# delldu/TransMVSNet

Hardware: AMD Instinct MI355X
Metric: depth maps/sec @ DTU 864x1152 N=5 (48/32/8 hyp); Abs depth L1 vs ref (higher is better)
Workload: dtype f32; 1 GPU; DTU 864x1152, N=5 views, cascade 48/32/8, B=1, hot path from FeatureNet outputs (FMT+pathway+stage glue+cost volume+CostRegNet+softmax/WTA); global_batch=1, parallelism=replica1, launch=hip_graph replay

## Files before the change

### transmvsnet_amd/csrc/common.h

```cpp
#pragma once

#include <hip/hip_runtime.h>
#include <stdint.h>

#include "../../include/transmvs.h"

#define TMVS_CHECK_LAUNCH()                                   \
  do {                                                        \
    hipError_t _e = hipGetLastError();                        \
    if (_e != hipSuccess) return TMVS_ERR_HIP;                \
  } while (0)

namespace tmvs {

constexpr int kWave = 64;

__device__ __forceinline__ float relu(float x) { return x > 0.f ? x : 0.f; }

__device__ __forceinline__ bool xcd_range_tap(int ntaps, int nblk, int& rb, int& k) {
  const int per = 8 * ntaps;
  const int grp = blockIdx.x / per, within = blockIdx.x % per;
  k = within / 8;
  rb = grp * 8 + within % 8;
  return rb < nblk;
}
static inline dim3 xcd_range_tap_grid(int ntaps, int nblk) { return dim3((unsigned)((nblk + 7) / 8 * 8 * ntaps)); }

__device__ __forceinline__ void chunk_row_coords(long v, int H, int W, int& b, int& y, int& x) {
  const long vl = v & ~63L;
  const unsigned lo = __builtin_amdgcn_readfirstlane((unsigned)vl);
  const unsigned hi = __builtin_amdgcn_readfirstlane((unsigned)((unsigned long)vl >> 32));
  const long vb = (long)(((unsigned long)hi << 32) | lo);
  const long t = vb / W;
  x = (int)(vb - t * W) + (int)(v - vb);
  y = (int)(t % H);
  b = (int)(t / H);
  while (x >= W) {
    x -= W;
    if (++y == H) {
      y = 0;
      ++b;
    }
  }
}

__device__ __forceinline__ void chunk_row_coords3(long v, int D, int H, int W, int& b, int& z, int& y, int& x) {
  const long vl = v & ~63L;
  const unsigned lo = __builtin_amdgcn_readfirstlane((unsigned)vl);
  const unsigned hi = __builtin_amdgcn_readfirstlane((unsigned)((unsigned long)vl >> 32));
  const long vb = (long)(((unsigned long)hi << 32) | lo);
  long t = vb / W;
  x = (int)(vb - t * W) + (int)(v - vb);
  y = (int)(t % H);
  t /= H;
  z = (int)(t % D);
  b = (int)(t / D);
  while (x >= W) {
    x -= W;
    if (++y == H) {
      y = 0;
      if (++z == D) {
        z = 0;
        ++b;
      }
    }
  }
}

template <int OFF>
__device__ __forceinline__ int xor_lane_dpp(int v) {
  if constexpr (OFF == 1) return __builtin_amdgcn_mov_dpp(v, 0xB1, 0xF, 0xF, false);
  else if constexpr (OFF == 2) return __builtin_amdgcn_mov_dpp(v, 0x4E, 0xF, 0xF, false);
  else if constexpr (OFF == 4)
    return __builtin_amdgcn_mov_dpp(__builtin_amdgcn_mov_dpp(v, 0x141, 0xF, 0xF, false), 0x1B, 0xF, 0xF, false);
  else if constexpr (OFF == 8)
    return __builtin_amdgcn_mov_dpp(__builtin_amdgcn_mov_dpp(v, 0x140, 0xF, 0xF, false), 0x141, 0xF, 0xF, false);
  else if constexpr (OFF == 16) return __builtin_amdgcn_ds_swizzle(v, 0x1F | (16 << 10));
  else return __shfl_xor(v, 32, 64);
}
template <int OFF>
__device__ __forceinline__ double xor_add_dpp(double x) {
  const int lo = xor_lane_dpp<OFF>(__double2loint(x)), hi = xor_lane_dpp<OFF>(__double2hiint(x));
  return x + __hiloint2double(hi, lo);
}
__device__ __forceinline__ double wave_xor_sum_dpp(double x) {
  x = xor_add_dpp<32>(x);
  x = xor_add_dpp<16>(x);
  x = xor_add_dpp<8>(x);
  x = xor_add_dpp<4>(x);
  x = xor_add_dpp<2>(x);
  return xor_add_dpp<1>(x);
}

template <typename T>
__device__ __forceinline__ double strided_sum(const T* __restrict__ p, long j0, long n, long step, size_t stride,
                                              double s) {
  constexpr int kBatch = 8;
  long j = j0;
  for (; j + (kBatch - 1) * step < n; j += kBatch * step) {
    T t[kBatch];
#pragma unroll
    for (int u = 0; u < kBatch; ++u) t[u] = p[(size_t)(j + u * step) * stride];
#pragma unroll
    for (int u = 0; u < kBatch; ++u) s += (double)t[u];
  }
  for (; j < n; j += step) s += (double)p[(size_t)j * stride];
  return s;
}

__device__ __forceinline__ int xcd_remap(int bid, int nblk) {
  const int xcd = bid & 7;
  const int q = nblk >> 3, r = nblk & 7;
  const int base = (xcd < r) ? xcd * (q + 1) : r * (q + 1) + (xcd - r) * q;
  return base + (bid >> 3);
}

constexpr int kRsrcWord3 = 0x00020000;
constexpr unsigned kOffOut = 0x80000000u;
__device__ __forceinline__ __amdgpu_buffer_rsrc_t raw_rsrc(const void* base, unsigned bytes) {
  return __builtin_amdgcn_make_buffer_rsrc(const_cast<void*>(base), (short)0, (int)bytes, kRsrcWord3);
}
__device__ __forceinline__ float buf_load_f32(__amdgpu_buffer_rsrc_t r, unsigned off) {
  return __uint_as_float(__builtin_amdgcn_raw_buffer_load_b32(r, (int)off, 0, 0));
}
typedef float floatx4_t __attribute__((ext_vector_type(4)));
__device__ __forceinline__ floatx4_t buf_load_f32x4(__amdgpu_buffer_rsrc_t r, unsigned off) {
  return __builtin_bit_cast(floatx4_t, __builtin_amdgcn_raw_buffer_load_b128(r, (int)off, 0, 0));
}

template <int D, typename PutProb>
__device__ __forceinline__ int softmax_first_max(const float (&x)[D], PutProb put_prob, float& best) {
  float m = x[0];
#pragma unroll
  for (int d = 1; d < D; ++d) m = fmaxf(m, x[d]);
  float s = 0.f;
#pragma unroll
  for (int d = 0; d < D; ++d) s = s + expf(x[d] - m);
  const float lse = logf(s);
  best = -1.f;
  int bi = 0;
#pragma unroll
  for (int d = 0; d < D; ++d) {
    const float pr = expf((x[d] - m) - lse);
    put_prob(d, pr);
    if (pr > best) {
      best = pr;
      bi = d;
    }
  }
  return bi;
}

}
```

### transmvsnet_amd/csrc/costreg.hip

```cpp
#include "common.h"

#include <utility>

namespace tmvs {

typedef float floatx4 __attribute__((ext_vector_type(4)));

struct Vec4 {
  float v[4];
  __device__ __forceinline__ void load(const float* p) {
    const float4 t = *reinterpret_cast<const float4*>(p);
    v[0] = t.x;
    v[1] = t.y;
    v[2] = t.z;
    v[3] = t.w;
  }
  __device__ __forceinline__ void zero() { v[0] = v[1] = v[2] = v[3] = 0.f; }
};

struct Buf {
  __amdgpu_buffer_rsrc_t r;
  __device__ __forceinline__ Buf(const float* base, uint32_t nbytes)
      : r(__builtin_amdgcn_make_buffer_rsrc(const_cast<float*>(base), (short)0, (int)nbytes, 0x00020000)) {}
  static constexpr int kOOB = (int)0x80000000u;
// ... 261 lines not shown
  auto chunk = [&](int ch, auto more_c) {
    constexpr bool MORE = decltype(more_c)::value;
    if (MORE && KDSKIP && kd_lo > kd_hi) fetch(ch + 1);
    if constexpr (KDSKIP) {
#pragma unroll 1
      for (int kd = kd_lo; kd <= kd_hi; ++kd)
#pragma unroll
        for (int k9 = 0; k9 < 9; ++k9) {
          if (k9 + 2 < 9) {
            wload(ch, kd * 9 + k9 + 2, aw[(k9 + 2) % 3]);
          } else {
            if (kd < kd_hi)
              wload(ch, kd * 9 + k9 + 2, aw[(k9 + 2) % 3]);
            else if (MORE)
              wload(ch + 1, kd_lo * 9 + k9 - 7, aw[(k9 + 2) % 3]);
          }
          if (MORE && k9 == 6 && kd == kd_hi) fetch(ch + 1);
          if (k9 == 0) bload(kd, k9 / 3, k9 % 3, bw[k9 & 1]);
          if (k9 + 1 < 9) bload(kd, (k9 + 1) / 3, (k9 + 1) % 3, bw[(k9 + 1) & 1]);
          tap_mfma(aw[k9 % 3], bw[k9 & 1]);
        }
    } else {
#pragma unroll
      for (int tap = 0; tap < 27; ++tap) {
        if (tap + 2 < 27)
          wload(ch, tap + 2, aw[(tap + 2) % 3]);
        else if (MORE)
          wload(ch + 1, tap - 25, aw[(tap + 2) % 3]);
        if (MORE && tap == 24) fetch(ch + 1);
        if (tap == 0) bload(tap / 9, (tap / 3) % 3, tap % 3, bw[tap & 1]);
        if (tap + 1 < 27) bload((tap + 1) / 9, ((tap + 1) / 3) % 3, (tap + 1) % 3, bw[(tap + 1) & 1]);
        tap_mfma(aw[tap % 3], bw[tap & 1]);
      }
    }
    if (MORE) {
      __syncthreads();
      commit();
      __syncthreads();
    }
  };
#pragma unroll 1
  for (int ch = 0; ch + 1 < NCH; ++ch) chunk(ch, std::true_type{});
  chunk(NCH - 1, std::false_type{});
  }
  const int ow = ow0 + col;
  if (ow >= g.Wo) return;
  const size_t out_n = (size_t)n * g.Do * g.Ho * g.Wo;
#pragma unroll
  for (int m = 0; m < MBW; ++m) {
    const int co = (mb0 + m) * 16 + kgrp * 4;
    const float4 al = *reinterpret_cast<const float4*>(alpha + co);
    const float4 sh = *reinterpret_cast<const float4*>(shift + co);
#pragma unroll
    for (int r = 0; r < NBW; ++r) {
      const int rr = rg * NBW + r;
      const int od = od0 + rr / TH, oh = oh0 + rr % TH;
      if (od >= g.Do || oh >= g.Ho) continue;
      *reinterpret_cast<float4*>(y + (out_n + ((size_t)od * g.Ho + oh) * g.Wo + ow) * COUT + co) =
          bn_act4(acc[r][m], al, sh, g.lo);
    }
  }
}

template <int CIN, int COUT, int TDI, int THI>
__global__ __launch_bounds__(256) void deconv3d_lds_kernel(const float* __restrict__ x,
                                                           const float* __restrict__ wpk,
                                                           const float* __restrict__ alpha,
                                                           const float* __restrict__ shift,
                                                           const float* __restrict__ skip, float* __restrict__ y,
                                                           Geo g) {
  constexpr int CK = 16, PL = 4;
  constexpr int MG = COUT / 16;
  constexpr int NBW = TDI * THI / 4;
  constexpr int LW = 17, LH = THI + 1, LD = TDI + 1;
  constexpr int NVOX = LD * LH * LW;
  static_assert((TDI * THI) % 4 == 0, "tile");
  static_assert(CIN % 16 == 0 && COUT % 16 == 0, "16-channel input chunks, 16-channel output blocks");
  __shared__ __attribute__((aligned(16))) float tile[NVOX * 16];
  __shared__ __attribute__((aligned(16))) float wts[27 * 16 * 16];

  const int nws = (g.Wi + 15) / 16, nhs = (g.Hi + THI - 1) / THI, nds = (g.Di + TDI - 1) / TDI;
  const int wg = xcd_remap(blockIdx.x, gridDim.x);
  const int mg = wg % MG;
  const TileCoord c = tile_coord(wg / MG, nws, nhs, nds, THI, TDI);
  const int n = c.n, mw0 = c.w0, mh0 = c.h0, md0 = c.d0;
  const int lane = threadIdx.x & 63, wv = threadIdx.x >> 6;
  const int col = lane & 15, kgrp = lane >> 4;
  const size_t in_n = (size_t)n * g.Di * g.Hi * g.Wi;

  floatx4 acc[NBW][8];
#pragma unroll
  for (int r = 0; r < NBW; ++r)
#pragma unroll
    for (int cls = 0; cls < 8; ++cls) acc[r][cls] = floatx4{0.f, 0.f, 0.f, 0.f};

#pragma unroll 1
  for (int ch = 0; ch < CIN / CK; ++ch) {
    if (ch) __syncthreads();
    for (int idx = threadIdx.x; idx < NVOX * PL; idx += 256) {
      const int vox = idx / PL, q = idx - vox * PL;
      const int lw = vox % LW, rest = vox / LW, lh = rest % LH, ld = rest / LH;
      const int iw = mw0 + lw, ih = mh0 + lh, id = md0 + ld;
      float4 v = make_float4(0.f, 0.f, 0.f, 0.f);
      if (iw < g.Wi && ih < g.Hi && id < g.Di)
        v = *reinterpret_cast<const float4*>(x + (in_n + ((size_t)id * g.Hi + ih) * g.Wi + iw) * CIN + ch * CK + 4 * q);
      *reinterpret_cast<float4*>(swz16(tile, vox, q)) = v;
    }
    stage_weights16<COUT, CIN>(wts, wpk, mg * 16, ch * CK);
    __syncthreads();
#pragma unroll
    for (int cls = 0; cls < 8; ++cls) {
#pragma unroll
      for (int i = 0; i < deconv_class_taps(cls); ++i) {
        const DeconvTap t = deconv_class_tap(cls, i);
        Vec4 a;
        a.load(swz16(wts + t.tap * 256, col, kgrp));
#pragma unroll
        for (int r = 0; r < NBW; ++r) {
          const int rr = wv * NBW + r;
          const int mdl = rr / THI, mhl = rr - mdl * THI;
          Vec4 b;
          const int lvox = ((mdl + (t.off >> 2)) * LH + mhl + ((t.off >> 1) & 1)) * LW + col + (t.off & 1);
          b.load(swz16(tile, lvox, kgrp));
#pragma unroll
          for (int j = 0; j < PL; ++j)
            acc[r][cls] = __builtin_amdgcn_mfma_f32_16x16x4f32(a.v[j], b.v[j], acc[r][cls], 0, 0, 0);
        }
      }
    }
  }
  const size_t out_n = (size_t)n * g.Do * g.Ho * g.Wo;
  const int mw = mw0 + col;
  if (mw >= g.Wi) return;
  const int co = mg * 16 + kgrp * 4;
  const float4 al = *reinterpret_cast<const float4*>(alpha + co);
  const float4 sh = *reinterpret_cast<const float4*>(shift + co);
#pragma unroll
  for (int r = 0; r < NBW; ++r) {
    const int rr = wv * NBW + r;
    const int md = md0 + rr / THI, mh = mh0 + rr % THI;
    if (md >= g.Di || mh >= g.Hi) continue;
#pragma unroll
    for (int cls = 0; cls < 8; ++cls) {
      const int od = 2 * md + (cls >> 2), oh = 2 * mh + ((cls >> 1) & 1), ow = 2 * mw + (cls & 1);
      const size_t o = (out_n + ((size_t)od * g.Ho + oh) * g.Wo + ow) * COUT + co;
      const float4 s = skip ? *reinterpret_cast<const float4*>(skip + o) : make_float4(0.f, 0.f, 0.f, 0.f);
      *reinterpret_cast<float4*>(y + o) = add4(s, bn_act4(acc[r][cls], al, sh, g.lo));
    }
  }
}

constexpr int kDChunk = 8;

constexpr int kProbCols = 62;
typedef float float2_v __attribute__((ext_vector_type(2)));

__device__ __forceinline__ float lane_from_left(float v) {
  return __int_as_float(__builtin_amdgcn_update_dpp(0, __float_as_int(v), 0x138, 0xF, 0xF, false));
}
__device__ __forceinline__ float lane_from_right(float v) {
  return __int_as_float(__builtin_amdgcn_update_dpp(0, __float_as_int(v), 0x130, 0xF, 0xF, false));
}

__global__ __launch_bounds__(256) void conv0_kernel(const float* __restrict__ x, float* __restrict__ y, int D, int H,
                                                    int W, const float* __restrict__ wt,
                                                    const float* __restrict__ alpha,
                                                    const float* __restrict__ shift, float lo) {
  const int HW = H * W;
  const int nseg = (W + kProbCols - 1) / kProbCols, nrow = (H + 3) / 4, ndc = (D + kDChunk - 1) / kDChunk;
  int lb = xcd_remap(blockIdx.x, gridDim.x);
  const int seg = lb % nseg;
  lb /= nseg;
  const int rowb = lb % nrow;
  lb /= nrow;
  const int dc = lb % ndc;
  const int n = lb / ndc;
  const int lane = threadIdx.x & 63;
  const int h = rowb * 4 + (threadIdx.x >> 6);
  if (h >= H) return;
  const int w = seg * kProbCols + lane - 1;
  const bool writes = lane >= 1 && lane <= kProbCols && w < W;
  const int d0 = dc * kDChunk, d1 = min(D, d0 + kDChunk);
  const __amdgpu_buffer_rsrc_t rx = raw_rsrc(x + (size_t)n * D * HW, (unsigned)(D * HW * 4));
  float* yp = y + ((size_t)n * D * HW + (size_t)h * W + w) * 8;
  const unsigned offw = (unsigned)w < (unsigned)W ? (unsigned)w * 4u : kOffOut;
  unsigned offh[3];
#pragma unroll
  for (int k = 0; k < 3; ++k) offh[k] = (unsigned)(h - 1 + k) < (unsigned)H ? (unsigned)((h - 1 + k) * W) * 4u : kOffOut;
  auto load_raw = [&](int d, float (&o)[3]) {
    const unsigned offd = (unsigned)d < (unsigned)D ? (unsigned)d * (unsigned)HW * 4u : kOffOut;
#pragma unroll
    for (int kh = 0; kh < 3; ++kh) {
      const unsigned off = offd | offh[kh] | offw;
      o[kh] = buf_load_f32(rx, (offd + offh[kh] + offw) | (off & kOffOut));
    }
  };
  auto expand = [&](const float (&r)[3], float (&o)[3][3]) {
#pragma unroll
    for (int kh = 0; kh < 3; ++kh) {
      o[kh][0] = lane_from_left(r[kh]);
      o[kh][1] = r[kh];
      o[kh][2] = lane_from_right(r[kh]);
    }
  };
  float al[8], sh[8];
#pragma unroll
  for (int c = 0; c < 8; ++c) {
    al[c] = alpha[c];
    sh[c] = shift[c];
  }
  float win[3][3][3];
  auto step = [&](int d, float (&raw)[3]) {
    expand(raw, win[2]);
    load_raw(d + 2, raw);
    const float* wk = wt;
    float2_v a[4] = {{0.f, 0.f}, {0.f, 0.f}, {0.f, 0.f}, {0.f, 0.f}};
#pragma unroll
    for (int t = 0; t < 27; ++t) {
      const float xv = win[t / 9][(t / 3) % 3][t % 3];
#pragma unroll
      for (int cp = 0; cp < 4; ++cp)
        a[cp] = __builtin_elementwise_fma(*reinterpret_cast<const float2_v*>(wk + t * 8 + 2 * cp), float2_v{xv, xv},
                                          a[cp]);
    }
    float o[8];
#pragma unroll
    for (int cp = 0; cp < 4; ++cp) {
      o[2 * cp] = act(fmaf(a[cp].x, al[2 * cp], sh[2 * cp]), lo);
      o[2 * cp + 1] = act(fmaf(a[cp].y, al[2 * cp + 1], sh[2 * cp + 1]), lo);
    }
    if (writes) {
      float4* q = reinterpret_cast<float4*>(yp + (size_t)d * HW * 8);
      q[0] = make_float4(o[0], o[1], o[2], o[3]);
      q[1] = make_float4(o[4], o[5], o[6], o[7]);
    }
#pragma unroll
    for (int kh = 0; kh < 3; ++kh)
#pragma unroll
      for (int k = 0; k < 3; ++k) {
        win[0][kh][k] = win[1][kh][k];
        win[1][kh][k] = win[2][kh][k];
      }
  };
  float ra[3];
  load_raw(d0 - 1, ra);
  expand(ra, win[0]);
  load_raw(d0, ra);
  expand(ra, win[1]);
  load_raw(d0 + 1, ra);
  for (int d = d0; d < d1; ++d) step(d, ra);
}


template <int NR, typename Emit>
__device__ __forceinline__ void prob_walk_rows(__amdgpu_buffer_rsrc_t rx, int w, int h, int D, int H, int W, int d0,
                                               const float* __restrict__ wt, Emit emit) {
  constexpr int NL = NR + 2;
  d0 = __builtin_amdgcn_readfirstlane(d0);
  const unsigned offw = (unsigned)w < (unsigned)W ? (unsigned)w * 32u : kOffOut;
  auto load_plane = [&](int i, float4 (&o)[NL][2]) {
#pragma unroll
    for (int j = 0; j < NL; ++j) {
      const int ih = h - 1 + j;
      const unsigned offr = ((unsigned)i < (unsigned)D && (unsigned)ih < (unsigned)H)
                                ? ((unsigned)i * (unsigned)H + (unsigned)ih) * (unsigned)W * 32u
                                : kOffOut;
      const unsigned off = (offr + offw) | ((offr | offw) & kOffOut);
      const floatx4 u = buf_load_f32x4(rx, off);
      const floatx4 v = buf_load_f32x4(rx, off + 16u);
      o[j][0] = make_float4(u[0], u[1], u[2], u[3]);
      o[j][1] = make_float4(v[0], v[1], v[2], v[3]);
    }
  };
  float2_v c12[NR];
#pragma unroll
  for (int r = 0; r < NR; ++r) c12[r] = float2_v{0.f, 0.f};
  auto plane = [&](int i, const float4 (&p)[NL][2]) {
    float acc_next[NR];
#pragma unroll
    for (int r = 0; r < NR; ++r) acc_next[r] = 0.f;
#pragma unroll
    for (int kh = 0; kh < 3; ++kh) {
      int wo = kh * 72;
      asm volatile("" : "+s"(wo));
      const float* wk = wt + __builtin_amdgcn_readfirstlane(wo);
#pragma unroll
      for (int r = 0; r < NR; ++r) {
        const int j = r + kh;
        const float xc[8] = {p[j][0].x, p[j][0].y, p[j][0].z, p[j][0].w, p[j][1].x, p[j][1].y, p[j][1].z, p[j][1].w};
#pragma unroll
        for (int kw = 0; kw < 3; ++kw) {
#pragma unroll
          for (int c = 0; c < 8; ++c) {
            const float xv = kw == 0 ? lane_from_left(xc[c]) : kw == 1 ? xc[c] : lane_from_right(xc[c]);
            const float2_v wp = *reinterpret_cast<const float2_v*>(wk + 2 * (kw * 8 + c));
            acc_next[r] = fmaf(wk[48 + kw * 8 + c], xv, acc_next[r]);
            c12[r] = __builtin_elementwise_fma(wp, float2_v{xv, xv}, c12[r]);
          }
        }
        asm volatile("" : "+v"(acc_next[r]), "+v"(c12[r]));
      }
    }
#pragma unroll
    for (int r = 0; r < NR; ++r) {
      if (i - 1 >= d0) emit(r, i - 1, c12[r].y);
      c12[r] = float2_v{acc_next[r], c12[r].x};
    }
  };
  float4 pa[NL][2], pb[NL][2];
  load_plane(d0 - 1, pa);
#pragma unroll
  for (int j = 0; j < kDChunk + 2; j += 2) {
    const int i = d0 - 1 + j;
    load_plane(i + 1, pb);
    plane(i, pa);
    load_plane(i + 2, pa);
    plane(i + 1, pb);
  }
}

template <int NR>
__global__ __launch_bounds__(256) void prob_kernel(const float* __restrict__ x, float* __restrict__ y, int D, int H,
                                                   int W, const float* __restrict__ wt) {
  const int HW = H * W;
  const int nseg = (W + kProbCols - 1) / kProbCols, nrow = (H + 4 * NR - 1) / (4 * NR), ndc = (D + kDChunk - 1) / kDChunk;
  int lb = xcd_remap(blockIdx.x, gridDim.x);
  const int seg = lb % nseg;
  lb /= nseg;
  const int rowb = lb % nrow;
  lb /= nrow;
  const int dc = lb % ndc;
  const int n = lb / ndc;
  const int lane = threadIdx.x & 63;
  const int h = (rowb * 4 + (threadIdx.x >> 6)) * NR;
  if (h >= H) return;
  const int w = seg * kProbCols + lane - 1;
  const bool writes = lane >= 1 && lane <= kProbCols && w < W;
  const int d0 = dc * kDChunk, d1 = min(D, d0 + kDChunk);
  const __amdgpu_buffer_rsrc_t rx = raw_rsrc(x + (size_t)n * D * HW * 8, (unsigned)(D * HW * 32));
  float* yn = y + (size_t)n * D * HW + (size_t)h * W + w;
  prob_walk_rows<NR>(rx, w, h, D, H, W, d0, wt, [&](int r, int d, float v) {
    if (d < d1 && writes && h + r < H) yn[(size_t)d * HW + (size_t)r * W] = v;
  });
}

template <int D, int NR>
__global__ __launch_bounds__(64 * (D / kDChunk)) void prob_wta_rows_kernel(
    const float* __restrict__ x, const float* __restrict__ wt, const float* __restrict__ hyp, int H, int W, float lo,
    float hi, float* __restrict__ prob, float* __restrict__ depth, float* __restrict__ depth_raw,
    float* __restrict__ conf) {
  constexpr int NW = D / kDChunk;
  __shared__ float lg[NR][D * 64];
  const int HW = H * W;
  const int nseg = (W + kProbCols - 1) / kProbCols, nrow = (H + NR - 1) / NR;
  int lb = xcd_remap(blockIdx.x, gridDim.x);
  const int seg = lb % nseg;
  lb /= nseg;
  const int h0 = (lb % nrow) * NR;
  const int n = lb / nrow;
  const int lane = threadIdx.x & 63, wv = threadIdx.x >> 6;
  const int d0 = wv * kDChunk;
  const int w = seg * kProbCols + lane - 1;
  const bool writes = lane >= 1 && lane <= kProbCols && w < W;
  const __amdgpu_buffer_rsrc_t rx = raw_rsrc(x + (size_t)n * D * HW * 8, (unsigned)(D * HW * 32));
  prob_walk_rows<NR>(rx, w, h0, D, H, W, d0, wt, [&](int r, int d, float v) { lg[r][d * 64 + lane] = v; });
  __syncthreads();
  if (!writes) return;
  for (int r = wv; r < NR; r += NW) {
    const int h = h0 + r;
    if (h >= H) break;
    float xl[D];
#pragma unroll
    for (int d = 0; d < D; ++d) xl[d] = lg[r][d * 64 + lane];
    const size_t base = (size_t)n * D * HW + (size_t)h * W + w;
    float best;
    const int bi = softmax_first_max<D>(xl, [&](int d, float pr) { prob[base + (size_t)d * HW] = pr; }, best);
    const size_t o = (size_t)n * HW + (size_t)h * W + w;
    const float dr = hyp[base + (size_t)bi * HW];
    depth_raw[o] = dr;
    depth[o] = fminf(fmaxf(dr, lo), hi);
    conf[o] = best;
  }
}

template <int TD, int TH>
__global__ __launch_bounds__(256) __attribute__((amdgpu_waves_per_eu(2))) void conv3d_c16_kernel(const float* __restrict__ x, const float* __restrict__ wpk,
                                                         const float* __restrict__ alpha,
                                                         const float* __restrict__ shift, float* __restrict__ y, Geo g,
                                                         int ntiles) {
  constexpr int C = 16, PL = 4, NWV = 4, NBW = TD * TH / NWV, NTH = NWV * 64;
  static_assert(TD * TH % NWV == 0, "rows split evenly over the waves");
  constexpr int LW = 18, LH = TH + 2, LD = TD + 2;
  constexpr int NVOX = LD * LH * LW;
  constexpr int NLD = (NVOX * 4 + NTH - 1) / NTH;
  __shared__ __attribute__((aligned(16))) float tile[NVOX * 16];
  __shared__ __attribute__((aligned(16))) float wts[27 * 16 * 16];
  const int nws = (g.Wo + 15) / 16, nhs = (g.Ho + TH - 1) / TH, nds = (g.Do + TD - 1) / TD;
  const int lane = threadIdx.x & 63, wv = threadIdx.x >> 6;
  const int col = lane & 15, kgrp = lane >> 4;
  const TileRange tr(ntiles);
  if (tr.idle()) return;
  auto coord = [&](int t) { return tile_coord(t, nws, nhs, nds, TH, TD); };
  float4 pf[NLD];
  auto fetch = [&](int t) {
    const TileCoord c = coord(t);
    const size_t in_n = (size_t)c.n * g.Di * g.Hi * g.Wi;
#pragma unroll
    for (int k = 0; k < NLD; ++k) {
      const int idx = threadIdx.x + NTH * k;
      const int vox = idx >> 2, q = idx & 3;
      const int lw = vox % LW, rest = vox / LW, lh = rest % LH, ld = rest / LH;
      const int iw = c.w0 - 1 + lw, ih = c.h0 - 1 + lh, id = c.d0 - 1 + ld;
      pf[k] = make_float4(0.f, 0.f, 0.f, 0.f);
      if (vox < NVOX && (unsigned)iw < (unsigned)g.Wi && (unsigned)ih < (unsigned)g.Hi && (unsigned)id < (unsigned)g.Di)
        pf[k] = *reinterpret_cast<const float4*>(x + (in_n + ((size_t)id * g.Hi + ih) * g.Wi + iw) * C + 4 * q);
    }
  };
  auto commit = [&]() {
#pragma unroll
    for (int k = 0; k < NLD; ++k) {
      const int idx = threadIdx.x + NTH * k;
      const int vox = idx >> 2, q = idx & 3;
      if (vox < NVOX) *reinterpret_cast<float4*>(swz16(tile, vox, q)) = pf[k];
    }
  };
  stage_weights16<C, C>(wts, wpk, 0, 0);
  const float4 al = *reinterpret_cast<const float4*>(alpha + kgrp * 4);
  const float4 sh = *reinterpret_cast<const float4*>(shift + kgrp * 4);
  int t = tr.first();
  if (t < tr.end) {
    fetch(t);
    commit();
  }
  __syncthreads();
  for (; t < tr.end; t += tr.step) {
    const TileCoord c = coord(t);
    const int tn = t + tr.step;
    if (tn < tr.end) fetch(tn);
    floatx4 acc[NBW];
#pragma unroll
    for (int r = 0; r < NBW; ++r) acc[r] = floatx4{0.f, 0.f, 0.f, 0.f};
#pragma unroll
    for (int tap = 0; tap < 27; ++tap) {
      const int kd = tap / 9, kh = (tap / 3) % 3, kw = tap % 3;
      Vec4 a;
      a.load(swz16(wts + tap * 256, col, kgrp));
      Vec4 b[NBW];
#pragma unroll
      for (int r = 0; r < NBW; ++r) {
        const int rr = wv * NBW + r;
        const int odl = rr / TH, ohl = rr - odl * TH;
        const int lvox = ((odl + kd) * LH + ohl + kh) * LW + col + kw;
        b[r].load(swz16(tile, lvox, kgrp));
      }
#pragma unroll
      for (int j = 0; j < PL; ++j)
#pragma unroll
        for (int r = 0; r < NBW; ++r)
          acc[r] = __builtin_amdgcn_mfma_f32_16x16x4f32(a.v[j], b[r].v[j], acc[r], 0, 0, 0);
      if (tap % (NBW > 2 ? 3 : 9) == (NBW > 2 ? 2 : 8)) __builtin_amdgcn_sched_barrier(0);
    }
    const int ow = c.w0 + col;
    const size_t out_n = (size_t)c.n * g.Do * g.Ho * g.Wo;
#pragma unroll
    for (int r = 0; r < NBW; ++r) {
      const int rr = wv * NBW + r;
      const int od = c.d0 + rr / TH, oh = c.h0 + rr % TH;
      if (ow >= g.Wo || od >= g.Do || oh >= g.Ho) continue;
      *reinterpret_cast<float4*>(y + (out_n + ((size_t)od * g.Ho + oh) * g.Wo + ow) * C + kgrp * 4) =
          bn_act4(acc[r], al, sh, g.lo);
// ... 460 lines not shown
      constexpr int s1 = s + 1, ch1 = s1 / 14, i1 = s1 % 14;
      constexpr bool next = s1 < 14 * NCH, next0 = next && deconv_stream_tap(0, i1).cls >= 0;
      if constexpr (next0) a[s1 & 1][0].load(wts[ch1] + deconv_stream_tap(0, i1).tap * 256 + woff);
      if constexpr (next) a[s1 & 1][1].load(wts[ch1] + deconv_stream_tap(1, i1).tap * 256 + woff);
      if constexpr (s < 8) bload(1, s);
      if constexpr (s < 8) sk[s] = sb.ld4(so[s]);
      if constexpr (s >= 8 && s < 8 + NLD) fetch1(fn, s - 8);
#pragma unroll
      for (int j = 0; j < PL; ++j) {
        if constexpr (t0.cls >= 0)
          acc[t0.cls] = __builtin_amdgcn_mfma_f32_16x16x4f32(a[s & 1][0].v[j], b[ch][t0.off].v[j], acc[t0.cls], 0, 0, 0);
        acc[t1.cls] = __builtin_amdgcn_mfma_f32_16x16x4f32(a[s & 1][1].v[j], b[ch][t1.off].v[j], acc[t1.cls], 0, 0, 0);
      }
      __builtin_amdgcn_sched_group_barrier(0x100, (next0 ? 1 : 0) + (next ? 1 : 0) + (s < 8 ? 1 : 0), 0);
      __builtin_amdgcn_sched_group_barrier(0x008, t0.cls >= 0 ? 2 * PL : PL, 0);
      if constexpr (ch == NCH - 1 && i >= 1 && deconv_class_done(i - 1) >= 0)
        epilogue(std::integral_constant<int, deconv_class_done(i - 1)>{});
      __builtin_amdgcn_sched_barrier(0);
    });
    epilogue(std::integral_constant<int, deconv_class_done(13)>{});
    __syncthreads();
    commit();
    __syncthreads();
  }
}

template <typename K>
static int persistent_cap(K kernel) {
  return persistent_grid(kernel, 1L << 40);
}

constexpr int kC16pMinTilesNum = 3, kC16pMinTilesDen = 2;

template <int TDI, int THI>
static int launch_deconv_c16p(const float* x, const float* w, const float* al, const float* sh, const float* skip,
                              float* y, int B, const Geo& g, hipStream_t st, int max_wgs = 0) {
  return launch_persistent(deconv3d_c16p_kernel<TDI, THI>, tile_count(B, g.Di, g.Hi, g.Wi, TDI, THI), max_wgs, st, x, w, al,
                           sh, skip, y, g);
}

template <int CIN, int COUT, int TDI, int THI>
static int launch_deconv(const float* x, const float* w, const float* al, const float* sh, const float* skip,
                         float* y, int B, const Geo& g, hipStream_t st) {
  const long nblk = tile_count(B, g.Di, g.Hi, g.Wi, TDI, THI) * (COUT / 16);
  hipLaunchKernelGGL((deconv3d_lds_kernel<CIN, COUT, TDI, THI>), dim3((unsigned)nblk), dim3(256), 0, st, x, w,
                     al, sh, skip, y, g);
  TMVS_CHECK_LAUNCH();
  return TMVS_OK;
}

static int conv_dispatch(const float* x, int B, int cin, int d, int h, int w, const float* wpk, const float* al,
                         const float* sh, int cout, int stride, float* y, hipStream_t st, float lo = 0.f) {
  const Geo g = Geo::conv(d, h, w, stride, lo);
  if ((long long)d * h * w * cin * 4 >= (1LL << 31)) return TMVS_ERR_SHAPE;
  constexpr int kKdSkipMaxDo = 2;
  const bool kdskip = g.Do <= kKdSkipMaxDo;
  constexpr bool KD = true, TAPOUT = true;
  using Conv3Tile = LdsTile<2, 2, 2, 2>;
  using Conv4Tile = LdsTile<2, 2, 2, 2>;
  using Conv4TileKd = LdsTile<2, 4, 2, 1>;
  using Conv5Tile = LdsTile<1, 2, 4, 4>;
  using Conv6Tile = LdsTile<1, 2, 4, 4>;
  int (*launch)(const float*, const float*, const float*, const float*, float*, int, const Geo&, hipStream_t) = nullptr;
  if (stride == 1) {
    if (cin == 16 && cout == 16)
      launch = launch_conv_c16<2, 4>;
    else if (cin == 32 && cout == 32)
      launch = kdskip ? launch_conv<32, 32, 1, Conv4TileKd, KD> : launch_conv<32, 32, 1, Conv4Tile>;
    else if (cin == 64 && cout == 64)
      launch = kdskip ? launch_conv<64, 64, 1, Conv6Tile, KD> : launch_conv<64, 64, 1, Conv6Tile>;
  } else {
    if (cin == 8 && cout == 16)
      launch = launch_conv_s2c8_tile<2, 2>;
    else if (cin == 16 && cout == 32)
      launch = kdskip ? launch_conv<16, 32, 2, Conv3Tile, KD> : launch_conv<16, 32, 2, Conv3Tile>;
    else if (cin == 32 && cout == 64)
      launch = launch_conv<32, 64, 2, Conv5Tile, false, TAPOUT>;
  }
  return launch ? launch(x, wpk, al, sh, y, B, g, st) : TMVS_ERR_SHAPE;
}

enum class Route { kAuto, kGeneric, kPersistent };

static int deconv_dispatch(const float* x, int B, int cin, int d, int h, int w, const float* wpk, const float* al,
                           const float* sh, int cout, const float* skip, float* y, hipStream_t st, float lo = 0.f,
                           Route route = Route::kAuto, int max_wgs = 0) {
  const Geo g = Geo::deconv(d, h, w, lo);
  const bool even = g.Di % 2 == 0;
  int (*launch)(const float*, const float*, const float*, const float*, const float*, float*, int, const Geo&,
                hipStream_t) = nullptr;
  if (cin == 64 && cout == 32)
    launch = even ? launch_deconv<64, 32, 2, 2> : launch_deconv<64, 32, 1, 4>;
  else if (cin == 32 && cout == 16)
    launch = even ? launch_deconv<32, 16, 2, 2> : launch_deconv<32, 16, 1, 4>;
  else if (cin == 16 && cout == 8)
    launch = even ? launch_deconv_c8<2, 2> : launch_deconv_c8<1, 4>;
  if (cin == 32 && cout == 16 && route != Route::kGeneric) {
    const bool fits = (long long)g.Do * g.Ho * g.Wo * cout * 4 < (1LL << 31);
    const int tdi = even ? 2 : 1, thi = even ? 2 : 4;
    const long ntiles = tile_count(B, d, h, w, tdi, thi);
    const int cap = even ? persistent_cap(deconv3d_c16p_kernel<2, 2>) : persistent_cap(deconv3d_c16p_kernel<1, 4>);
    if (route == Route::kPersistent && !fits) return TMVS_ERR_SHAPE;
    if (route == Route::kPersistent || (fits && ntiles * kC16pMinTilesDen >= (long)cap * kC16pMinTilesNum))
      return even ? launch_deconv_c16p<2, 2>(x, wpk, al, sh, skip, y, B, g, st, max_wgs)
                  : launch_deconv_c16p<1, 4>(x, wpk, al, sh, skip, y, B, g, st, max_wgs);
  } else if (route == Route::kPersistent) {
    return TMVS_ERR_SHAPE;
  }
  return launch ? launch(x, wpk, al, sh, skip, y, B, g, st) : TMVS_ERR_SHAPE;
}


}

using namespace tmvs;

extern "C" int tmvs_conv3d_bn_relu(const float* x, int batch, int cin, int d, int h, int w, const float* wpk,
                                   const float* alpha, const float* shift, int cout, int stride, float* y,
                                   void* stream) {
  if (!x || !wpk || !alpha || !shift || !y || batch <= 0 || d <= 0 || h <= 0 || w <= 0) return TMVS_ERR_ARG;
  if (stride != 1 && stride != 2) return TMVS_ERR_ARG;
  return conv_dispatch(x, batch, cin, d, h, w, wpk, alpha, shift, cout, stride, y, (hipStream_t)stream);
}

extern "C" int tmvs_deconv3d_bn_relu_add(const float* x, int batch, int cin, int d, int h, int w, const float* wpk,
                                         const float* alpha, const float* shift, int cout, const float* skip,
                                         float* y, void* stream) {
  if (!x || !wpk || !alpha || !shift || !skip || !y || batch <= 0 || d <= 0 || h <= 0 || w <= 0)
    return TMVS_ERR_ARG;
  return deconv_dispatch(x, batch, cin, d, h, w, wpk, alpha, shift, cout, skip, y, (hipStream_t)stream);
}

extern "C" int tmvs_deconv3d_bn_relu_add_generic(const float* x, int batch, int cin, int d, int h, int w,
                                                 const float* wpk, const float* alpha, const float* shift, int cout,
                                                 const float* skip, float* y, void* stream) {
  if (!x || !wpk || !alpha || !shift || !skip || !y || batch <= 0 || d <= 0 || h <= 0 || w <= 0)
    return TMVS_ERR_ARG;
  return deconv_dispatch(x, batch, cin, d, h, w, wpk, alpha, shift, cout, skip, y, (hipStream_t)stream, 0.f,
                         Route::kGeneric);
}

extern "C" int tmvs_deconv3d_bn_relu_add_persistent(const float* x, int batch, int cin, int d, int h, int w,
                                                    const float* wpk, const float* alpha, const float* shift,
                                                    int cout, const float* skip, float* y, int max_workgroups,
                                                    void* stream) {
  if (!x || !wpk || !alpha || !shift || !skip || !y || batch <= 0 || d <= 0 || h <= 0 || w <= 0 || max_workgroups < 0)
    return TMVS_ERR_ARG;
  return deconv_dispatch(x, batch, cin, d, h, w, wpk, alpha, shift, cout, skip, y, (hipStream_t)stream, 0.f,
                         Route::kPersistent, max_workgroups);
}

static int launch_conv0(const float* x, float* y, int batch, int D, int H, int W, const float* wt, const float* al,
                        const float* sh, float lo, hipStream_t st) {
  const dim3 grid((unsigned)(((W + kProbCols - 1) / kProbCols) * ((H + 3) / 4) * batch * ((D + kDChunk - 1) / kDChunk)));
  hipLaunchKernelGGL(conv0_kernel, grid, dim3(256), 0, st, x, y, D, H, W, wt, al, sh, lo);
  TMVS_CHECK_LAUNCH();
  return TMVS_OK;
}

static int launch_prob(const float* x, float* y, int batch, int D, int H, int W, const float* wt, hipStream_t st) {
  constexpr int NR = 1;
  const dim3 grid((unsigned)(((W + kProbCols - 1) / kProbCols) * ((H + 4 * NR - 1) / (4 * NR)) * batch *
                             ((D + kDChunk - 1) / kDChunk)));
  hipLaunchKernelGGL(prob_kernel<NR>, grid, dim3(256), 0, st, x, y, D, H, W, wt);
  TMVS_CHECK_LAUNCH();
  return TMVS_OK;
}

__device__ float kUnitAlpha[64] = {1.f, 1.f, 1.f, 1.f, 1.f, 1.f, 1.f, 1.f, 1.f, 1.f, 1.f, 1.f, 1.f, 1.f, 1.f, 1.f,
                                   1.f, 1.f, 1.f, 1.f, 1.f, 1.f, 1.f, 1.f, 1.f, 1.f, 1.f, 1.f, 1.f, 1.f, 1.f, 1.f,
                                   1.f, 1.f, 1.f, 1.f, 1.f, 1.f, 1.f, 1.f, 1.f, 1.f, 1.f, 1.f, 1.f, 1.f, 1.f, 1.f,
                                   1.f, 1.f, 1.f, 1.f, 1.f, 1.f, 1.f, 1.f, 1.f, 1.f, 1.f, 1.f, 1.f, 1.f, 1.f, 1.f};
__device__ float kZeroShift[64];

extern "C" int tmvs_conv3d_mfma(const float* x, int batch, int cin, int d, int h, int w, const float* wpk, int cout,
                                int stride, int transposed, const float* skip, float* y, void* stream) {
  if (!x || !wpk || !y || batch <= 0 || d <= 0 || h <= 0 || w <= 0) return TMVS_ERR_ARG;
  if (transposed ? stride != 2 : (stride != 1 && stride != 2)) return TMVS_ERR_ARG;
  if (skip && !transposed) return TMVS_ERR_ARG;
  int dev = 0;
  if (hipGetDevice(&dev) != hipSuccess || dev < 0 || dev >= 64) return TMVS_ERR_HIP;
  static const float* unit[64][2];
  if (!unit[dev][0]) {
    void *a, *b;
    if (hipGetSymbolAddress(&a, HIP_SYMBOL(kUnitAlpha)) != hipSuccess ||
        hipGetSymbolAddress(&b, HIP_SYMBOL(kZeroShift)) != hipSuccess)
      return TMVS_ERR_HIP;
    unit[dev][1] = (const float*)b;
    unit[dev][0] = (const float*)a;
  }
  const float *al = unit[dev][0], *sh = unit[dev][1];
  const float lo = -__builtin_huge_valf();
  hipStream_t st = (hipStream_t)stream;
  if (!transposed && stride == 1 && cin == 1 && cout == 8) {
    if ((long long)d * h * w * 32 >= (1LL << 31)) return TMVS_ERR_SHAPE;
    return launch_conv0(x, y, batch, d, h, w, wpk, al, sh, lo, st);
  }
  if (!transposed && stride == 1 && cin == 8 && cout == 1) {
    if ((long long)d * h * w * 32 >= (1LL << 31)) return TMVS_ERR_SHAPE;
    return launch_prob(x, y, batch, d, h, w, wpk, st);
  }
  if (transposed) return deconv_dispatch(x, batch, cin, d, h, w, wpk, al, sh, cout, skip, y, st, lo);
  return conv_dispatch(x, batch, cin, d, h, w, wpk, al, sh, cout, stride, y, st, lo);
}

static size_t align_up(size_t v) { return (v + 255) & ~(size_t)255; }

extern "C" size_t tmvs_costregnet_workspace(int batch, int depth, int height, int width, int base_ch) {
  const size_t v0 = (size_t)batch * depth * height * width;
  const size_t v1 = v0 / 8, v2 = v0 / 64, v3 = v0 / 512;
  const size_t c = (size_t)base_ch;
  size_t bytes = 0;
  bytes += align_up(v0 * c * 4);
  bytes += align_up(v1 * 2 * c * 4) * 2;
  bytes += align_up(v2 * 4 * c * 4) * 2;
  bytes += align_up(v3 * 8 * c * 4) * 2;
  bytes += align_up(v2 * 4 * c * 4);
  bytes += align_up(v1 * 2 * c * 4);
  bytes += align_up(v0 * c * 4);
  return bytes;
}

static int costregnet_trunk(const float* x, int batch, int depth, int height, int width, const TmvsCostRegWeights* w,
                            void* workspace, size_t workspace_bytes, hipStream_t st, float** x11_out,
                            float** c0_out) {
  if (!x || !w || !workspace || batch <= 0) return TMVS_ERR_ARG;
  if (depth % 8 || height % 8 || width % 8) return TMVS_ERR_SHAPE;
  if (w->base_ch != 8) return TMVS_ERR_SHAPE;
  if ((long long)depth * height * width * 32 >= (1LL << 31)) return TMVS_ERR_SHAPE;
  for (int i = 0; i < 11; ++i)
    if (!w->w[i]) return TMVS_ERR_ARG;
  for (int i = 0; i < 10; ++i)
    if (!w->alpha[i] || !w->shift[i]) return TMVS_ERR_ARG;
  if (workspace_bytes < tmvs_costregnet_workspace(batch, depth, height, width, w->base_ch)) return TMVS_ERR_ARG;
  const int c = w->base_ch;
  const size_t v0 = (size_t)batch * depth * height * width;
  const size_t v1 = v0 / 8, v2 = v0 / 64, v3 = v0 / 512;
  char* ws = (char*)workspace;
  auto take = [&](size_t n) {
    float* p = (float*)ws;
    ws += align_up(n * 4);
    return p;
  };
  float* c0 = take(v0 * c);
  float* c1 = take(v1 * 2 * c);
  float* c2 = take(v1 * 2 * c);
  float* c3 = take(v2 * 4 * c);
  float* c4 = take(v2 * 4 * c);
  float* c5 = take(v3 * 8 * c);
  float* c6 = take(v3 * 8 * c);
  float* x7 = take(v2 * 4 * c);
  float* x9 = take(v1 * 2 * c);
  float* x11 = take(v0 * c);
  const int D0 = depth, H0 = height, W0 = width;
  const int D1 = D0 / 2, H1 = H0 / 2, W1 = W0 / 2;
  const int D2 = D1 / 2, H2 = H1 / 2, W2 = W1 / 2;
  const int D3 = D2 / 2, H3 = H2 / 2, W3 = W2 / 2;
  int rc;
  if ((rc = launch_conv0(x, c0, batch, D0, H0, W0, w->w[0], w->alpha[0], w->shift[0], 0.f, st))) return rc;
  if ((rc = conv_dispatch(c0, batch, c, D0, H0, W0, w->w[1], w->alpha[1], w->shift[1], 2 * c, 2, c1, st))) return rc;
  if ((rc = conv_dispatch(c1, batch, 2 * c, D1, H1, W1, w->w[2], w->alpha[2], w->shift[2], 2 * c, 1, c2, st)))
    return rc;
  if ((rc = conv_dispatch(c2, batch, 2 * c, D1, H1, W1, w->w[3], w->alpha[3], w->shift[3], 4 * c, 2, c3, st)))
    return rc;
  if ((rc = conv_dispatch(c3, batch, 4 * c, D2, H2, W2, w->w[4], w->alpha[4], w->shift[4], 4 * c, 1, c4, st)))
    return rc;
  if ((rc = conv_dispatch(c4, batch, 4 * c, D2, H2, W2, w->w[5], w->alpha[5], w->shift[5], 8 * c, 2, c5, st)))
    return rc;
  if ((rc = conv_dispatch(c5, batch, 8 * c, D3, H3, W3, w->w[6], w->alpha[6], w->shift[6], 8 * c, 1, c6, st)))
    return rc;
  if ((rc = deconv_dispatch(c6, batch, 8 * c, D3, H3, W3, w->w[7], w->alpha[7], w->shift[7], 4 * c, c4, x7, st)))
    return rc;
  if ((rc = deconv_dispatch(x7, batch, 4 * c, D2, H2, W2, w->w[8], w->alpha[8], w->shift[8], 2 * c, c2, x9, st)))
    return rc;
  if ((rc = deconv_dispatch(x9, batch, 2 * c, D1, H1, W1, w->w[9], w->alpha[9], w->shift[9], c, c0, x11, st)))
    return rc;
  *x11_out = x11;
  *c0_out = c0;
  return TMVS_OK;
}

extern "C" int tmvs_costregnet(const float* x, int batch, int depth, int height, int width,
                               const TmvsCostRegWeights* w, void* workspace, size_t workspace_bytes, float* logits,
                               void* stream) {
  if (!logits) return TMVS_ERR_ARG;
  hipStream_t st = (hipStream_t)stream;
  float *x11, *c0;
  int rc;
  if ((rc = costregnet_trunk(x, batch, depth, height, width, w, workspace, workspace_bytes, st, &x11, &c0))) return rc;
  return launch_prob(x11, logits, batch, depth, height, width, w->w[10], st);
}

extern "C" int tmvs_costregnet_wta(const float* x, const float* hyp, int batch, int depth, int height, int width,
                                   const TmvsCostRegWeights* w, void* workspace, size_t workspace_bytes,
                                   float clamp_lo, float clamp_hi, float* prob, float* depth_out, float* depth_raw,
                                   float* conf, void* stream) {
  if (!hyp || !prob || !depth_out || !depth_raw || !conf) return TMVS_ERR_ARG;
  switch (depth) {
    case 8: case 16: case 24: case 32: case 48: case 64: break;
    default: return TMVS_ERR_SHAPE;
  }
  hipStream_t st = (hipStream_t)stream;
  float *x11, *c0;
  int rc;
  if ((rc = costregnet_trunk(x, batch, depth, height, width, w, workspace, workspace_bytes, st, &x11, &c0))) return rc;
  if (depth > 32) {
    if ((rc = launch_prob(x11, c0, batch, depth, height, width, w->w[10], st))) return rc;
// ... 20 lines not shown
```

Baseline: 304.7 depth_maps/s.

## Restructure conv0 with multi-row register blocking, deep prefetch, buffer stores; trim prob edge FMAs

The first CostRegNet conv kernel now has each wave compute two output rows, so input rows loaded for the vertical stencil are shared between them. The depth loop is fully unrolled with loads issued several planes ahead, and stores go through raw buffer stores with out-of-bounds offsets instead of branches. The prob kernel skips FMAs whose results are thrown away at the first and last planes of a chunk. The cost is much higher register use from the unrolled prefetch window, plus fewer blocks in the grid.

```diff
diff --git a/transmvsnet_amd/csrc/common.h b/transmvsnet_amd/csrc/common.h
--- a/transmvsnet_amd/csrc/common.h
+++ b/transmvsnet_amd/csrc/common.h
@@ -127,6 +127,10 @@
 __device__ __forceinline__ floatx4_t buf_load_f32x4(__amdgpu_buffer_rsrc_t r, unsigned off) {
   return __builtin_bit_cast(floatx4_t, __builtin_amdgcn_raw_buffer_load_b128(r, (int)off, 0, 0));
 }
+typedef unsigned uintx4_t __attribute__((ext_vector_type(4)));
+__device__ __forceinline__ void buf_store_f32x4(__amdgpu_buffer_rsrc_t r, unsigned off, floatx4_t v) {
+  __builtin_amdgcn_raw_buffer_store_b128(__builtin_bit_cast(uintx4_t, v), r, (int)off, 0, 0);
+}
 
 template <int D, typename PutProb>
 __device__ __forceinline__ int softmax_first_max(const float (&x)[D], PutProb put_prob, float& best) {
diff --git a/transmvsnet_amd/csrc/costreg.hip b/transmvsnet_amd/csrc/costreg.hip
--- a/transmvsnet_amd/csrc/costreg.hip
+++ b/transmvsnet_amd/csrc/costreg.hip
@@ -437,6 +437,7 @@
 
 constexpr int kDChunk = 8;
 
+constexpr int kConv0Rows = 2, kConv0Ahead = 6;
 constexpr int kProbCols = 62;
 typedef float float2_v __attribute__((ext_vector_type(2)));
 
@@ -446,13 +447,18 @@
 __device__ __forceinline__ float lane_from_right(float v) {
   return __int_as_float(__builtin_amdgcn_update_dpp(0, __float_as_int(v), 0x130, 0xF, 0xF, false));
 }
+
+__device__ __forceinline__ unsigned off_add(unsigned a, unsigned b) { return (a + b) | ((a | b) & kOffOut); }
 
 __global__ __launch_bounds__(256) void conv0_kernel(const float* __restrict__ x, float* __restrict__ y, int D, int H,
                                                     int W, const float* __restrict__ wt,
                                                     const float* __restrict__ alpha,
                                                     const float* __restrict__ shift, float lo) {
+  constexpr int NR = kConv0Rows, PF = kConv0Ahead;
+  constexpr int NL = NR + 2, NP = kDChunk + 2;
+  static_assert(PF >= 2 && PF <= NP, "prefetch distance");
   const int HW = H * W;
-  const int nseg = (W + kProbCols - 1) / kProbCols, nrow = (H + 3) / 4, ndc = (D + kDChunk - 1) / kDChunk;
+  const int nseg = (W + kProbCols - 1) / kProbCols, nrow = (H + 4 * NR - 1) / (4 * NR), ndc = (D + kDChunk - 1) / kDChunk;
   int lb = xcd_remap(blockIdx.x, gridDim.x);
   const int seg = lb % nseg;
   lb /= nseg;
@@ -461,79 +467,87 @@
   const int dc = lb % ndc;
   const int n = lb / ndc;
   const int lane = threadIdx.x & 63;
-  const int h = rowb * 4 + (threadIdx.x >> 6);
+  const int h = (rowb * 4 + (threadIdx.x >> 6)) * NR;
   if (h >= H) return;
   const int w = seg * kProbCols + lane - 1;
   const bool writes = lane >= 1 && lane <= kProbCols && w < W;
-  const int d0 = dc * kDChunk, d1 = min(D, d0 + kDChunk);
+  const int d0 = __builtin_amdgcn_readfirstlane(dc * kDChunk);
+  const int nd = min(D - d0, kDChunk);
   const __amdgpu_buffer_rsrc_t rx = raw_rsrc(x + (size_t)n * D * HW, (unsigned)(D * HW * 4));
-  float* yp = y + ((size_t)n * D * HW + (size_t)h * W + w) * 8;
-  const unsigned offw = (unsigned)w < (unsigned)W ? (unsigned)w * 4u : kOffOut;
-  unsigned offh[3];
-#pragma unroll
-  for (int k = 0; k < 3; ++k) offh[k] = (unsigned)(h - 1 + k) < (unsigned)H ? (unsigned)((h - 1 + k) * W) * 4u : kOffOut;
-  auto load_raw = [&](int d, float (&o)[3]) {
-    const unsigned offd = (unsigned)d < (unsigned)D ? (unsigned)d * (unsigned)HW * 4u : kOffOut;
-#pragma unroll
-    for (int kh = 0; kh < 3; ++kh) {
-      const unsigned off = offd | offh[kh] | offw;
-      o[kh] = buf_load_f32(rx, (offd + offh[kh] + offw) | (off & kOffOut));
-    }
-  };
-  auto expand = [&](const float (&r)[3], float (&o)[3][3]) {
-#pragma unroll
-    for (int kh = 0; kh < 3; ++kh) {
-      o[kh][0] = lane_from_left(r[kh]);
-      o[kh][1] = r[kh];
-      o[kh][2] = lane_from_right(r[kh]);
-    }
-  };
+  const __amdgpu_buffer_rsrc_t ry = raw_rsrc(y + ((size_t)n * D + d0) * HW * 8, (unsigned)(nd * HW * 32));
+  unsigned offi[NL], offo[NR];
+#pragma unroll
+  for (int j = 0; j < NL; ++j)
+    offi[j] = ((unsigned)(h - 1 + j) < (unsigned)H && (unsigned)w < (unsigned)W) ? (unsigned)((h - 1 + j) * W + w) * 4u
+                                                                                 : kOffOut;
+#pragma unroll
+  for (int r = 0; r < NR; ++r) offo[r] = (writes && h + r < H) ? (unsigned)((h + r) * W + w) * 32u : kOffOut;
   float al[8], sh[8];
 #pragma unroll
   for (int c = 0; c < 8; ++c) {
     al[c] = alpha[c];
     sh[c] = shift[c];
   }
-  float win[3][3][3];
-  auto step = [&](int d, float (&raw)[3]) {
-    expand(raw, win[2]);
-    load_raw(d + 2, raw);
-    const float* wk = wt;
-    float2_v a[4] = {{0.f, 0.f}, {0.f, 0.f}, {0.f, 0.f}, {0.f, 0.f}};
-#pragma unroll
-    for (int t = 0; t < 27; ++t) {
-      const float xv = win[t / 9][(t / 3) % 3][t % 3];
-#pragma unroll
-      for (int cp = 0; cp < 4; ++cp)
-        a[cp] = __builtin_elementwise_fma(*reinterpret_cast<const float2_v*>(wk + t * 8 + 2 * cp), float2_v{xv, xv},
-                                          a[cp]);
-    }
-    float o[8];
-#pragma unroll
-    for (int cp = 0; cp < 4; ++cp) {
-      o[2 * cp] = act(fmaf(a[cp].x, al[2 * cp], sh[2 * cp]), lo);
-      o[2 * cp + 1] = act(fmaf(a[cp].y, al[2 * cp + 1], sh[2 * cp + 1]), lo);
-    }
-    if (writes) {
-      float4* q = reinterpret_cast<float4*>(yp + (size_t)d * HW * 8);
-      q[0] = make_float4(o[0], o[1], o[2], o[3]);
-      q[1] = make_float4(o[4], o[5], o[6], o[7]);
-    }
-#pragma unroll
-    for (int kh = 0; kh < 3; ++kh)
-#pragma unroll
-      for (int k = 0; k < 3; ++k) {
-        win[0][kh][k] = win[1][kh][k];
-        win[1][kh][k] = win[2][kh][k];
+  float raw[NP][NL], win[NP][NL][3];
+  auto request = [&](int k) {
+    const int i = d0 - 1 + k;
+    const unsigned offd = (unsigned)i < (unsigned)D ? (unsigned)i * (unsigned)HW * 4u : kOffOut;
+#pragma unroll
+    for (int j = 0; j < NL; ++j) raw[k][j] = buf_load_f32(rx, off_add(offi[j], offd));
+  };
+  auto expand = [&](int k) {
+#pragma unroll
+    for (int j = 0; j < NL; ++j) {
+      win[k][j][0] = lane_from_left(raw[k][j]);
+      win[k][j][1] = raw[k][j];
+      win[k][j][2] = lane_from_right(raw[k][j]);
+    }
+  };
+#pragma unroll
+  for (int k = 0; k <= PF; ++k) request(k);
+  expand(0);
+  expand(1);
+#pragma unroll
+  for (int p = 0; p < kDChunk; ++p) {
+    if (p + 1 + PF < NP) request(p + 1 + PF);
+    float2_v a[NR][4];
+#pragma unroll
+    for (int r = 0; r < NR; ++r)
+#pragma unroll
+      for (int cp = 0; cp < 4; ++cp) a[r][cp] = float2_v{0.f, 0.f};
+#pragma unroll
+    for (int kd = 0; kd < 3; ++kd) {
+      if (kd == 2) expand(p + 2);
+      int wo = kd * 72;
+      asm volatile("" : "+s"(wo));
+      const float* wk = wt + __builtin_amdgcn_readfirstlane(wo);
+#pragma unroll
+      for (int t = 0; t < 9; ++t) {
+#pragma unroll
+        for (int cp = 0; cp < 4; ++cp) {
+          const float2_v wp = *reinterpret_cast<const float2_v*>(wk + t * 8 + 2 * cp);
+#pragma unroll
+          for (int r = 0; r < NR; ++r) {
+            const float xv = win[p + kd][r + t / 3][t % 3];
+            a[r][cp] = __builtin_elementwise_fma(wp, float2_v{xv, xv}, a[r][cp]);
+          }
+        }
       }
-  };
-  float ra[3];
-  load_raw(d0 - 1, ra);
-  expand(ra, win[0]);
-  load_raw(d0, ra);
-  expand(ra, win[1]);
-  load_raw(d0 + 1, ra);
-  for (int d = d0; d < d1; ++d) step(d, ra);
+    }
+    const unsigned offp = p < nd ? (unsigned)p * (unsigned)HW * 32u : kOffOut;
+#pragma unroll
+    for (int r = 0; r < NR; ++r) {
+      float o[8];
+#pragma unroll
+      for (int cp = 0; cp < 4; ++cp) {
+        o[2 * cp] = act(fmaf(a[r][cp].x, al[2 * cp], sh[2 * cp]), lo);
+        o[2 * cp + 1] = act(fmaf(a[r][cp].y, al[2 * cp + 1], sh[2 * cp + 1]), lo);
+      }
+      const unsigned off = off_add(offo[r], offp);
+      buf_store_f32x4(ry, off, floatx4_t{o[0], o[1], o[2], o[3]});
+      buf_store_f32x4(ry, off + 16u, floatx4_t{o[4], o[5], o[6], o[7]});
+    }
+  }
 }
 
 
@@ -560,7 +574,9 @@
   float2_v c12[NR];
 #pragma unroll
   for (int r = 0; r < NR; ++r) c12[r] = float2_v{0.f, 0.f};
-  auto plane = [&](int i, const float4 (&p)[NL][2]) {
+  auto plane = [&](int j, const float4 (&p)[NL][2]) {
+    const int i = d0 - 1 + j;
+    const bool first = j == 0, last = j == kDChunk + 1, no_next = j >= kDChunk;
     float acc_next[NR];
 #pragma unroll
     for (int r = 0; r < NR; ++r) acc_next[r] = 0.f;
@@ -571,16 +587,19 @@
       const float* wk = wt + __builtin_amdgcn_readfirstlane(wo);
 #pragma unroll
       for (int r = 0; r < NR; ++r) {
-        const int j = r + kh;
-        const float xc[8] = {p[j][0].x, p[j][0].y, p[j][0].z, p[j][0].w, p[j][1].x, p[j][1].y, p[j][1].z, p[j][1].w};
+        const int l = r + kh;
+        const float xc[8] = {p[l][0].x, p[l][0].y, p[l][0].z, p[l][0].w, p[l][1].x, p[l][1].y, p[l][1].z, p[l][1].w};
 #pragma unroll
         for (int kw = 0; kw < 3; ++kw) {
 #pragma unroll
           for (int c = 0; c < 8; ++c) {
             const float xv = kw == 0 ? lane_from_left(xc[c]) : kw == 1 ? xc[c] : lane_from_right(xc[c]);
             const float2_v wp = *reinterpret_cast<const float2_v*>(wk + 2 * (kw * 8 + c));
-            acc_next[r] = fmaf(wk[48 + kw * 8 + c], xv, acc_next[r]);
-            c12[r] = __builtin_elementwise_fma(wp, float2_v{xv, xv}, c12[r]);
+            if (!no_next) acc_next[r] = fmaf(wk[48 + kw * 8 + c], xv, acc_next[r]);
+            if (last)
+              c12[r].y = fmaf(wp.y, xv, c12[r].y);
+            else if (!first)
+              c12[r] = __builtin_elementwise_fma(wp, float2_v{xv, xv}, c12[r]);
           }
         }
         asm volatile("" : "+v"(acc_next[r]), "+v"(c12[r]));
@@ -598,9 +617,9 @@
   for (int j = 0; j < kDChunk + 2; j += 2) {
     const int i = d0 - 1 + j;
     load_plane(i + 1, pb);
-    plane(i, pa);
+    plane(j, pa);
     load_plane(i + 2, pa);
-    plane(i + 1, pb);
+    plane(j + 1, pb);
   }
 }
 
@@ -1367,7 +1386,9 @@
 
 static int launch_conv0(const float* x, float* y, int batch, int D, int H, int W, const float* wt, const float* al,
                         const float* sh, float lo, hipStream_t st) {
-  const dim3 grid((unsigned)(((W + kProbCols - 1) / kProbCols) * ((H + 3) / 4) * batch * ((D + kDChunk - 1) / kDChunk)));
+  constexpr int NR = kConv0Rows;
+  const dim3 grid((unsigned)(((W + kProbCols - 1) / kProbCols) * ((H + 4 * NR - 1) / (4 * NR)) * batch *
+                             ((D + kDChunk - 1) / kDChunk)));
   hipLaunchKernelGGL(conv0_kernel, grid, dim3(256), 0, st, x, y, D, H, W, wt, al, sh, lo);
   TMVS_CHECK_LAUNCH();
   return TMVS_OK;
```

After: 307.6 depth_maps/s, median of 6. No clear change (+1.0%).
